# esheldon/ngmix

Measured on AMD Instinct MI355X. Metric: pixel-Gaussian evals/sec (render+loglike), 48×48×6-gauss stamps, 1/2/4/8 GPU, higher is better.
Workload: dtype f64

## Files before the change

### include/ngmix_hip.h

```cpp
#ifndef NGMIX_HIP_H
#define NGMIX_HIP_H

#include <stddef.h>
#include <stdint.h>

#ifdef __cplusplus
extern "C" {
#endif

#define NGMIX_OK 0
#define NGMIX_ERR_DET_TOO_LOW 1
#define NGMIX_ERR_T_TOO_LOW 2
#define NGMIX_ERR_G_RANGE 3
#define NGMIX_ERR_GTOT_ZERO 4
#define NGMIX_ERR_ELOGL_ZERO 5
#define NGMIX_ERR_ZERO_DIV 6
#define NGMIX_ERR_PIXELS_NOT_FILLED 7
#define NGMIX_ERR_HIP (-100)
#define NGMIX_ERR_BAD_ARG (-101)

#define NGMIX_FLAG_CEN_SHIFT 2
#define NGMIX_FLAG_NONPOS_FLUX 4
#define NGMIX_FLAG_NONPOS_SIZE 8
#define NGMIX_FLAG_LOW_DET 16
// ... 110 lines not shown
                            int nmom, double maxrad);
int ngmix_admom(const ngmix_admom_conf *conf, ngmix_gauss2d *wt,
                const ngmix_pixel *pixels, int64_t npix,
                ngmix_admom_result *res);
int ngmix_em_run(int kind, const ngmix_em_conf *conf, ngmix_pixel *pixels,
                 int64_t npix, double *sums, ngmix_gauss2d *gmix, int64_t ngauss,
                 ngmix_gauss2d *gmix_psf, int64_t npsf, ngmix_gauss2d *gmix_conv,
                 int fill_zero_weight, int32_t *numiter, double *frac_diff,
                 double *sky);
int ngmix_deriv_images(const double *gpars, const double *dcov, int64_t ngauss,
                       const double *vv, const double *uu, const double *area,
                       int64_t npix, double *out);


#define NGMIX_STAMP_IGNORE_ZERO_WEIGHT 1

typedef struct {
    int64_t pix_off;
    int32_t nrow, ncol;
    int32_t gm_off;
    int32_t ngauss;
    int32_t flags;
    int32_t npix_kept;
} ngmix_stamp;

#define NGMIX_BATCH_NO_SKIP 1
#define NGMIX_BATCH_EXACT 2
#define NGMIX_BATCH_TRACKED_LOADS 4
#define NGMIX_BATCH_RENDER_OVERWRITE 8

typedef struct {
    int64_t nstamps;
    const ngmix_stamp *stamps;
    const double *val;
    const double *ierr;
    const ngmix_jacobian *jac;
    int32_t max_ngauss;
    int32_t max_npix;
    int32_t any_masked;
    int32_t flags;
    int32_t max_nrow;
    int32_t max_ncol;
} ngmix_batch;

// ... 229 lines not shown
```

### ngmix_amd/_lib.py

```python
import ctypes
import os
import subprocess

import numpy as np

from . import gexceptions

_HERE = os.path.dirname(os.path.abspath(__file__))
_CSRC = os.path.join(_HERE, "csrc")
LIB_PATH = os.environ.get("NGMIX_HIP_LIB", os.path.join(_HERE, "libngmix_hip.so"))

OK = 0
ERR_DET_TOO_LOW = 1
ERR_T_TOO_LOW = 2
ERR_G_RANGE = 3
ERR_GTOT_ZERO = 4
ERR_ELOGL_ZERO = 5
ERR_ZERO_DIV = 6
ERR_PIXELS_NOT_FILLED = 7
ERR_HIP = -100
ERR_BAD_ARG = -101

_RANGE_MESSAGES = {
    ERR_DET_TOO_LOW: "det too low",
    ERR_T_TOO_LOW: "T too low",
    ERR_G_RANGE: "g >= 1",
    ERR_GTOT_ZERO: "gtot == 0",
    ERR_ELOGL_ZERO: "elogL == 0",
}

STAMP_IGNORE_ZERO_WEIGHT = 1
BATCH_NO_SKIP = 1
BATCH_EXACT = 2
BATCH_TRACKED_LOADS = 4
BATCH_RENDER_OVERWRITE = 8

GAUSS2D_DTYPE = np.dtype([
    ("p", "f8"), ("row", "f8"), ("col", "f8"),
    ("irr", "f8"), ("irc", "f8"), ("icc", "f8"), ("det", "f8"),
    ("norm_set", "i8"),
    ("drr", "f8"), ("drc", "f8"), ("dcc", "f8"), ("norm", "f8"), ("pnorm", "f8"),
])
PIXEL_DTYPE = np.dtype([
    ("u", "f8"), ("v", "f8"), ("area", "f8"),
    ("val", "f8"), ("ierr", "f8"), ("fdiff", "f8"),
])
COORD_DTYPE = np.dtype([("u", "f8"), ("v", "f8"), ("area", "f8")])
JACOBIAN_DTYPE = np.dtype([
    ("row0", "f8"), ("col0", "f8"), ("dvdrow", "f8"), ("dvdcol", "f8"),
    ("dudrow", "f8"), ("dudcol", "f8"), ("det", "f8"), ("scale", "f8"),
# ... 338 lines not shown
```

### ngmix_amd/batch.py

```python
import ctypes

import numpy as np

from . import _lib


def _torch():
    import torch
    return torch


def _stream():
    torch = _torch()
    raw = getattr(torch._C, "_cuda_getCurrentRawStream", None)
    if raw is not None:
        return ctypes.c_void_p(raw(torch.cuda.current_device()))
    return ctypes.c_void_p(torch.cuda.current_stream().cuda_stream)


class _on_device(object):

    def __init__(self, dev):
        torch = _torch()
        idx = dev.index if hasattr(dev, "index") else int(dev)
# ... 119 lines not shown
        flat = self.data.detach().cpu().numpy()
        return flat.reshape(-1).view(_lib.GAUSS2D_DTYPE).reshape(
            self.n, self.ngauss).copy()

    def clone(self):
        return GMixBatch(self.data.clone(), self.n, self.ngauss)

    def select(self, index):
        torch = _torch()
        idx = torch.as_tensor(np.ascontiguousarray(index, dtype=np.int64),
                              device=self.device)
        rows = self.data.reshape(self.n, self.ngauss * 13)[idx]
        return GMixBatch(rows.reshape(-1, 13).contiguous(), idx.numel(), self.ngauss)


class StampBatch(object):

    def __init__(self, val, ierr, jac, nrow, ncol, pix_off, ignore_zero_weight,
                 npix_kept=None):
        torch = _torch()
        self.val = val
        self.ierr = ierr
        self.jac = jac
        self.device = ierr.device if ierr is not None else jac.device
        self.n = int(jac.shape[0])
        self.nrow = np.ascontiguousarray(nrow, dtype=np.int32)
        self.ncol = np.ascontiguousarray(ncol, dtype=np.int32)
        self.pix_off = np.ascontiguousarray(pix_off, dtype=np.int64)
        izw = np.broadcast_to(np.asarray(ignore_zero_weight, dtype=bool), (self.n,))
        self.flags = np.where(izw, _lib.STAMP_IGNORE_ZERO_WEIGHT, 0).astype(np.int32)
        self.npix = self.nrow.astype(np.int64) * self.ncol
        self.tracked_loads = False
        self.max_npix = int(self.npix.max()) if self.n else 0
        self.total_pix = int(self.npix.sum())
        self._stamp_tables = {}
        self.npix_kept = self.npix.astype(np.int32).copy()
        if npix_kept is not None:
            self.npix_kept = np.ascontiguousarray(npix_kept, dtype=np.int32)
        elif ierr is not None and self.n:
            tab = self._make_table(self.npix_kept, 0, 0)
            with _on_device(self.device):
                st = _lib.lib().ngmix_count_kept_batch(
                    _dptr(tab), self.n, _dptr(self.ierr), _stream())
            _lib.check(st, "ngmix_count_kept_batch")
            host = tab.cpu().numpy().reshape(-1).view(_lib.STAMP_DTYPE)
            self.npix_kept = host["npix_kept"].copy()
        self.any_masked = bool(np.any(self.npix_kept != self.npix))

    @classmethod
    def from_images(cls, images, weights=None, jacobians=None,
                    ignore_zero_weight=True, device=None):
        torch = _torch()
        dev = _require_cuda(device)
        val = _as_device_f64(images, dev)
        if val.ndim == 2:
            val = val[None]
        n, nrow, ncol = val.shape
        if weights is None:
            ierr = torch.ones_like(val)
        else:
            w = _as_device_f64(weights, dev)
            if w.ndim == 2:
# ... 28 lines not shown
                               [o._ignore_zero_weight for o in obs_list], device=device)

    @classmethod
    def from_arrays(cls, imgs, weights, jac_records, ignore_zero_weight, device=None):
        torch = _torch()
        dev = _require_cuda(device)
        nrow = np.array([im.shape[0] for im in imgs], dtype=np.int32)
        ncol = np.array([im.shape[1] for im in imgs], dtype=np.int32)
        npix = nrow.astype(np.int64) * ncol
        off = np.concatenate([[0], np.cumsum(npix)[:-1]]).astype(np.int64)
        izw = np.array(ignore_zero_weight, dtype=bool)
        tot = int(npix.sum())
        n = len(imgs)
        host = np.empty(2 * tot + 8 * n + 4 * n)
        kept = np.empty(n, dtype=np.int32)
        for i in range(n):
            a, b = int(off[i]), int(off[i] + npix[i])
            host[a:b] = np.asarray(imgs[i], dtype="f8").ravel()
            w = np.asarray(weights[i], dtype="f8").ravel()
            host[tot + a:tot + b] = w
            kept[i] = np.count_nonzero(w > 0.0) if izw[i] else npix[i]
            host[2 * tot + 8 * i:2 * tot + 8 * i + 8] = \
                np.ascontiguousarray(jac_records[i]).view(np.float64).reshape(8)
        tab = np.zeros(n, dtype=_lib.STAMP_DTYPE)
        tab["pix_off"], tab["nrow"], tab["ncol"] = off, nrow, ncol
        tab["gm_off"] = np.arange(n, dtype=np.int32)
        tab["ngauss"] = 1
        tab["flags"] = np.where(izw, _lib.STAMP_IGNORE_ZERO_WEIGHT, 0)
        tab["npix_kept"] = kept
        host[2 * tot + 8 * n:] = tab.view(np.float64)
        dev_all = torch.from_numpy(host).to(dev)
        dval = dev_all[:tot]
        dw = dev_all[tot:2 * tot]
        djac = dev_all[2 * tot:2 * tot + 8 * n].reshape(n, 8)
        dtab = dev_all[2 * tot + 8 * n:].view(torch.int32).reshape(n, 8)
        with _on_device(dev):
            st = _lib.lib().ngmix_weight_to_ierr_batch(
                _dptr(dw), _dptr(dw), dw.numel(), _stream())
        _lib.check(st, "ngmix_weight_to_ierr_batch")
        sb = cls(dval, dw, djac, nrow, ncol, off, izw, npix_kept=kept)
        sb._stamp_tables[1] = dtab
        return sb

    @classmethod
    def from_stacked(cls, images, weights, jac_records, ignore_zero_weight=True,
                     device=None):
        torch = _torch()
        dev = _require_cuda(device)
        if isinstance(images, torch.Tensor):
            ok = (torch.float64, torch.float32)
            assert images.dtype in ok and weights.dtype in ok, "float64 or float32 stamps"
            n, nrow, ncol = images.shape
            assert weights.shape == images.shape, "image and weight must match"
            dval = images.to(dev, non_blocking=True).reshape(-1)
            dw = weights.to(dev, non_blocking=True).reshape(-1)
# ... 14 lines not shown
            return cls(dval, dw, djac, np.full(n, nrow), np.full(n, ncol),
                       np.arange(n, dtype=np.int64) * npix, ignore_zero_weight)
        images = np.asarray(images, dtype="f8")
        weights = np.asarray(weights, dtype="f8")
        n, nrow, ncol = images.shape
        assert weights.shape == images.shape, "image and weight must match"
        npix = nrow * ncol
        tot = n * npix
        jr = np.ascontiguousarray(jac_records)
        if jr.dtype.names is not None:
            jr = jr.view(np.float64)
        jr = jr.reshape(n, 8)
        izw = np.broadcast_to(np.asarray(ignore_zero_weight, dtype=bool), (n,))
        kept = np.where(izw, np.count_nonzero(weights.reshape(n, -1) > 0.0, axis=1),
                        npix).astype(np.int32)
        off = np.arange(n, dtype=np.int64) * npix
        tab = np.zeros(n, dtype=_lib.STAMP_DTYPE)
        tab["pix_off"], tab["nrow"], tab["ncol"] = off, nrow, ncol
        tab["gm_off"] = np.arange(n, dtype=np.int32)
        tab["ngauss"] = 1
        tab["flags"] = np.where(izw, _lib.STAMP_IGNORE_ZERO_WEIGHT, 0)
        tab["npix_kept"] = kept
        host = np.empty(2 * tot + 8 * n + 4 * n)
        host[:tot] = images.reshape(-1)
        host[tot:2 * tot] = weights.reshape(-1)
        host[2 * tot:2 * tot + 8 * n] = jr.reshape(-1)
        host[2 * tot + 8 * n:] = tab.view(np.float64)
        dev_all = torch.from_numpy(host).to(dev)
        dval = dev_all[:tot]
        dw = dev_all[tot:2 * tot]
        djac = dev_all[2 * tot:2 * tot + 8 * n].reshape(n, 8)
        dtab = dev_all[2 * tot + 8 * n:].view(torch.int32).reshape(n, 8)
        with _on_device(dev):
            st = _lib.lib().ngmix_weight_to_ierr_batch(
                _dptr(dw), _dptr(dw), dw.numel(), _stream())
        _lib.check(st, "ngmix_weight_to_ierr_batch")
        sb = cls(dval, dw, djac, np.full(n, nrow), np.full(n, ncol), off, izw, npix_kept=kept)
        sb._stamp_tables[1] = dtab
        return sb

    @classmethod
    def from_observations_geometry(cls, obs_list, device=None):
        dev = _require_cuda(device)
        nrow = np.array([o.image.shape[0] for o in obs_list], dtype=np.int32)
        ncol = np.array([o.image.shape[1] for o in obs_list], dtype=np.int32)
        npix = nrow.astype(np.int64) * ncol
        off = np.concatenate([[0], np.cumsum(npix)[:-1]]).astype(np.int64)
        jac = np.stack([o.jacobian.get_data().view(np.float64).reshape(8)
                        for o in obs_list])
        return cls(None, None, _as_device_f64(jac, dev), nrow, ncol, off, False)

    @staticmethod
# ... 57 lines not shown
        b = _lib.Batch()
        b.nstamps = self.n
        b.stamps = self.stamp_table(ngauss).data_ptr()
        if np.ndim(ngauss) != 0:
            ngauss = int(np.max(ngauss)) if self.n else 0
        b.val = self.val.data_ptr() if self.val is not None else None
        b.ierr = self.ierr.data_ptr() if self.ierr is not None else None
        b.jac = self.jac.data_ptr()
        b.max_ngauss = ngauss
        b.max_npix = self.max_npix
        b.any_masked = int(self.any_masked)
        b.max_nrow = int(self.nrow.max()) if self.n else 0
        b.max_ncol = int(self.ncol.max()) if self.n else 0
        b.flags = (_lib.BATCH_NO_SKIP if no_skip else 0) | \
            (_lib.BATCH_EXACT if exact else 0) | \
            (_lib.BATCH_TRACKED_LOADS if self.tracked_loads else 0)
        return b

    def _packed(self):
        if not hasattr(self, "_packed_layout"):
            start = np.concatenate([[0], np.cumsum(self.npix)[:-1]]) if self.n else \
                np.zeros(0, dtype=np.int64)
            self._packed_layout = bool(np.array_equal(self.pix_off, start))
        return self._packed_layout

    def kept_offsets(self):
        kept = self.npix_kept.astype(np.int64)
        return np.concatenate([[0], np.cumsum(kept)[:-1]]).astype(np.int64)

    def loglike(self, gm, out=None, status=None, no_skip=False, exact=False):
        torch = _torch()
# ... 429 lines not shown
```

### ngmix_amd/csrc/pixpass.hip

```cpp
#include <stdlib.h>

#include <type_traits>

#include "device_utils.hpp"
#include "launch.hpp"

namespace ngmix {

__constant__ double c_exp_table[16] = NGMIX_EXP_TABLE;
__constant__ double c_fexp_coef[12] = NGMIX_FEXP_COEF;

enum PassOp { OP_LOGLIKE = 0, OP_FDIFF = 1, OP_RENDER_FAST = 2,
              OP_RENDER_EXACT = 3, OP_S2N = 4 };

struct GaussLds {
    EvalGauss e;
    PixBox box;
};
static_assert(sizeof(GaussLds) == 64, "GaussLds");

struct LdsLayout {
    double *tab;
    double *red;
    int *ctl;
// ... 290 lines not shown
        "s_mov_b64 %0, exec\n\t"
        "s_and_b64 exec, exec, %3\n\t"
        "global_store_dwordx2 %1, %2, %4\n\t"
        "s_mov_b64 exec, %0"
        : "=&s"(save)
        : "v"(off), "v"(v), "s"(lanes), "s"(base)
        : "scc");
}

__device__ __forceinline__ void gload2_f64_if(double &d0, const void *base0, double &d1,
                                              const void *base1, unsigned off,
                                              int on_mask)
{
    unsigned long long save;
    asm volatile(
        "s_mov_b64 %2, exec\n\t"
        "s_and_b32 exec_lo, exec_lo, %4\n\t"
        "s_and_b32 exec_hi, exec_hi, %4\n\t"
        "global_load_dwordx2 %0, %3, %5\n\t"
        "global_load_dwordx2 %1, %3, %6\n\t"
        "s_mov_b64 exec, %2"
        : "+v"(d0), "+v"(d1), "=&s"(save)
        : "v"(off), "s"(on_mask), "s"(base0), "s"(base1)
        : "scc");
}

template <int N>
__device__ __forceinline__ void wait_vm(double &a, double &b)
{
    asm volatile("s_waitcnt vmcnt(%2)" : "+v"(a), "+v"(b) : "n"(N));
}

__device__ __forceinline__ void wait_vm_all(double &a, double &b, double &c, double &d,
                                            double &e, double &f, double &g, double &h)
{
    asm volatile("s_waitcnt vmcnt(0)"
                 : "+v"(a), "+v"(b), "+v"(c), "+v"(d), "+v"(e), "+v"(f), "+v"(g), "+v"(h));
}

template <int OP, bool MASKED, bool FAST, bool FULL, int TW, bool SKIP>
__device__ __forceinline__ void wave_tiles(
    const LdsLayout &L, const GaussFused *gf, const TileBox *gbox, const TileEnt *te,
    int ng,
    const ngmix_stamp &st, const double *__restrict__ sval,
    const double *__restrict__ sierr, bool masked, double *out, int64_t out_base,
    const ngmix_jacobian &jac, double (&pv)[FUSED_PF], double (&pe)[FUSED_PF],
    double &acc_ll, double &acc_sn, double &acc_sd, const int keep, const TileBox &ub)
{
    constexpr bool kNeedsVal = (OP == OP_LOGLIKE || OP == OP_FDIFF);
    constexpr bool kNeedsIerr = (OP != OP_RENDER_FAST);
    constexpr int TH = WAVE / TW;
    const bool overwrite = keep == 0;
    static_assert(!SKIP || OP == OP_RENDER_FAST, "the line skip is the render's");
    const int lane = threadIdx.x;
    const int lrow = lane / TW, lcol = lane % TW;
    const int nrow = st.nrow, ncol = st.ncol;
    const int ntx = (ncol + TW - 1) / TW;
    const int nty = (nrow + TH - 1) / TH;
    int ntiles = __builtin_amdgcn_readfirstlane(ntx * nty);
    constexpr bool full = FULL;
    const double cen_row = FAST ? gf[0].row : 0.0, cen_col = FAST ? gf[0].col : 0.0;
    const double olv =
// ... 30 lines not shown
    }
    const unsigned long long valid_mask = __builtin_amdgcn_ballot_w64(lane_valid);
    unsigned long long allmask = 0ull;
    int kc = 0;
    const FexpCoef K = load_fexp_coef(c_fexp_coef);

    auto prefetch = [&](int Tn, bool &inb_n, unsigned long long &rm_n, double &nval,
                        double &nierr) {
        if (full) {
            inb_n = true;
            int on;
            asm("s_sub_i32 %0, %1, %2\n\ts_ashr_i32 %0, %0, 31"
                : "=s"(on) : "s"(Tn), "s"(ntiles) : "scc");
            const unsigned off2 = lane_off + (unsigned)te[Tn].off;
            if (kNeedsVal && kNeedsIerr) {
                gload2_f64_if(nval, bval, nierr, bierr, off2, on);
            } else {
                if (kNeedsVal) gload_f64_if(nval, bval, off2, on);
                if (kNeedsIerr) gload_f64_if(nierr, bierr, off2, on);
                if (OP == OP_RENDER_FAST && !SKIP)
                    gload_f64_if(nval, bimg, off2, on & keep);
                if (SKIP) {
                    unsigned long long mr, mc;
                    asm("v_cmp_le_u32 %0, %1, %2"
                        : "=s"(mr)
                        : "v"((unsigned)(te[Tn].r0 + lrow - ub.r_lo)), "s"(ub.r_span));
                    asm("v_cmp_le_u32 %0, %1, %2"
                        : "=s"(mc) : "v"((unsigned)(te[Tn].c0 - ub.c_lo)), "s"(ub.c_span));
                    rm_n = mr & mc;
                    gload_f64_lanes(nval, bimg, off2, rm_n & (unsigned long long)(long long)on);
                }
            }
        } else {
            const int r0n = te[Tn].r0, c0n = te[Tn].c0;
            inb_n = (r0n < rlim) & (c0n < clim);
            if (SKIP)
                inb_n &= ((unsigned)(r0n + lrow - ub.r_lo) <= ub.r_span) &
                         ((unsigned)(c0n - ub.c_lo) <= ub.c_span);
            nval = 0.0;
            nierr = 0.0;
            if (inb_n) {
                const unsigned off2 = lane_off + (unsigned)te[Tn].off;
                if (kNeedsVal) nval = *(const double *)(bval + off2);
                if (kNeedsIerr) nierr = *(const double *)(bierr + off2);
                if (OP == OP_RENDER_FAST && !overwrite) nval = *(const double *)(bimg + off2);
            }
        }
    };

    constexpr int kLoadsPerTile = (kNeedsVal ? 1 : 0) + (kNeedsIerr ? 1 : 0) +
                                  (OP == OP_RENDER_FAST ? 1 : 0);
    auto compute = [&](auto nyounger, int Tc, bool inb, unsigned long long rm, double &pval,
                       double &pierr) {
        const double v = te[Tc].bv + olv, u = te[Tc].bu + olu;
        double dv = v, du = u;
        double v2 = dv * dv, u2 = du * du, vu = dv * du;
        double model = 0.0;

        for (int g0 = 0; g0 < ng; g0 += 32) {
// ... 95 lines not shown
    }
    while (T < ntiles) {
        compute(Y3{}, T, in0, rm0, va0, ie0);
        if (T + 1 < ntiles) compute(Y2{}, T + 1, in1, rm1, va1, ie1);
        prefetch(T + 4, in0, rm0, va0, ie0);
        prefetch(T + 5, in1, rm1, va1, ie1);
        if (T + 2 < ntiles) compute(Y3{}, T + 2, in2, rm2, va2, ie2);
        if (T + 3 < ntiles) compute(Y2{}, T + 3, in3, rm3, va3, ie3);
        prefetch(T + 6, in2, rm2, va2, ie2);
        prefetch(T + 7, in3, rm3, va3, ie3);
        T += 4;
    }
    if (full) wait_vm_all(va0, ie0, va1, ie1, va2, ie2, va3, ie3);
}

template <int OP, bool MASKED, int TW, bool LS = (OP == OP_RENDER_FAST)>
__device__ __forceinline__ void pixpass_wave_body(
    const ngmix_stamp *__restrict__ stamps, const double *__restrict__ val,
    const double *__restrict__ ierr, const ngmix_jacobian *__restrict__ jacs,
    ngmix_gauss2d *gmix, double *out, const int64_t *__restrict__ out_start,
    int32_t *status, int max_ngauss, int nchunks_cap, int no_skip, int tile_cap)
{
    extern __shared__ __attribute__((aligned(16))) char smem[];
    const LdsLayout L = carve(smem, max_ngauss, nchunks_cap, tile_cap);
    GaussFused *gf = (GaussFused *)L.gl;
    TileBox *gbox = (TileBox *)(gf + max_ngauss);
    TileEnt *te = (TileEnt *)L.tb;

    const int s = blockIdx.x;
    const ngmix_stamp st = stamps[s];
    const ngmix_jacobian jac = jacs[s];
    const int nrow = st.nrow, ncol = st.ncol, ng = st.ngauss;
    const int npix = nrow * ncol;
    ngmix_gauss2d *gm = gmix + st.gm_off;
    const double *sval = val + st.pix_off;
    const double *sierr = ierr + st.pix_off;
    const bool izw = (st.flags & NGMIX_STAMP_IGNORE_ZERO_WEIGHT) != 0;
    constexpr bool kNeedsVal = (OP == OP_LOGLIKE || OP == OP_FDIFF);
    const double area = jac.scale * jac.scale;
    const int lane = threadIdx.x;

    constexpr int TH = WAVE / TW;
    const int ntx = (ncol + TW - 1) / TW;
    const int nty = (nrow + TH - 1) / TH;
    const int ntiles = ntx * nty;
    for (int T = lane; T < ntiles + FUSED_SENTINELS; T += WAVE) {
        TileEnt e;
        if (T < ntiles) {
            const int ty = T / ntx, tx = T - ty * ntx;
            e.r0 = ty * TH;
            e.c0 = tx * TW;
            const double rd = (double)e.r0 - jac.row0, cd = (double)e.c0 - jac.col0;
            e.bv = fma(jac.dvdrow, rd, jac.dvdcol * cd);
            e.bu = fma(jac.dudrow, rd, jac.dudcol * cd);
            e.off = (e.r0 * ncol + e.c0) * 8;
// ... 19 lines not shown
    const int keep = (OP == OP_RENDER_FAST && !LS) ? (((no_skip >> 2) & 1) - 1) : -1;
    const bool full = (nrow % TH) == 0 && (ncol % TW) == 0 && !(no_skip & 2);
    double pv[FUSED_PF], pe[FUSED_PF];
#pragma unroll
    for (int t = 0; t < FUSED_PF; t++) {
        pv[t] = 0.0;
        pe[t] = 0.0;
    }
    if (full && ng > 0 && ntiles > 0 && !LS) {
        const unsigned lane_off = (unsigned)((lane / TW) * ncol + lane % TW) * 8u;
#pragma unroll
        for (int t = 0; t < FUSED_PF; t++) {
            const int on = __builtin_amdgcn_readfirstlane(-(int)(t < ntiles));
            const unsigned off = lane_off + (unsigned)te[t].off;
            if (kNeedsVal) gload_f64_if(pv[t], (const char *)sval, off, on);
            if (OP != OP_RENDER_FAST) gload_f64_if(pe[t], (const char *)sierr, off, on);
            if (OP == OP_RENDER_FAST)
                gload_f64_if(pv[t], (const char *)(out + st.pix_off), off, on & keep);
        }
    }

    const bool overwrite = OP == OP_RENDER_FAST && !LS && (no_skip & 4);
    const int stcode = lazy_norms<WAVE>(L, gm, ng);
    if (stcode != NGMIX_OK || (overwrite && ng == 0)) {
        asm volatile("s_waitcnt vmcnt(0)" ::: "memory");
        if (overwrite)
            for (int p = lane; p < npix; p += WAVE) out[st.pix_off + p] = 0.0;
        if (lane == 0) status[s] = stcode;
        return;
    }
    if (lane < 16) L.tab[lane] = c_exp_table[15 - lane];
// ... 32 lines not shown
        un.cmin = ubx[2];
        un.cmax = ubx[3];
        const TileBox t = tile_box(un, 1, TW);
        ub.r_lo = __builtin_amdgcn_readfirstlane(t.r_lo);
        ub.r_span = (unsigned)__builtin_amdgcn_readfirstlane((int)t.r_span);
        ub.c_lo = __builtin_amdgcn_readfirstlane(t.c_lo);
        ub.c_span = (unsigned)__builtin_amdgcn_readfirstlane((int)t.c_span);
    }
    const bool masked = MASKED && izw && st.npix_kept != npix;
    if (OP == OP_FDIFF && masked) build_rank_tables<WAVE>(L.cmask, L.cpre, sierr, npix);
    const int64_t out_base = (OP == OP_FDIFF) ? out_start[s] : 0;

    double acc_ll = 0.0, acc_sn = 0.0, acc_sd = 0.0;
    if (ng > 0) {
        if (fast && full)
            wave_tiles<OP, MASKED, true, true, TW, LS>(L, gf, gbox, te, ng, st, sval, sierr, masked,
                out, out_base, jac, pv, pe, acc_ll, acc_sn, acc_sd, keep, ub);
        else if (fast)
            wave_tiles<OP, MASKED, true, false, TW, LS>(L, gf, gbox, te, ng, st, sval, sierr, masked,
                out, out_base, jac, pv, pe, acc_ll, acc_sn, acc_sd, keep, ub);
        else if (full)
            wave_tiles<OP, MASKED, false, true, TW, LS>(L, gf, gbox, te, ng, st, sval, sierr, masked,
                out, out_base, jac, pv, pe, acc_ll, acc_sn, acc_sd, keep, ub);
        else
            wave_tiles<OP, MASKED, false, false, TW, LS>(L, gf, gbox, te, ng, st, sval, sierr, masked,
                out, out_base, jac, pv, pe, acc_ll, acc_sn, acc_sd, keep, ub);
    } else if (OP != OP_RENDER_FAST) {
        for (int p = lane; p < npix; p += WAVE) {
            const double pv = kNeedsVal ? sval[p] : 0.0, pe = sierr[p];
            if (masked && !(pe > 0.0)) continue;
            if (OP == OP_LOGLIKE) acc_ll = fma(pv * pv, pe * pe, acc_ll);
            if (OP == OP_FDIFF) {
                const int rank = masked ? kept_rank(L.cmask, L.cpre, p) : p;
                out[out_base + rank] = (0.0 - pv) * pe;
            }
        }
    }

    if (OP == OP_LOGLIKE) {
        double *red = L.red;
        const double r0_ = row16_total(acc_ll), r1_ = row16_total(acc_sn),
// ... 45 lines not shown
{
    pixpass_wave_body<OP, MASKED, TW, false>(stamps, val, ierr, jacs, gmix, out, out_start,
                                             status, max_ngauss, nchunks_cap, no_skip, tile_cap);
}

template <int OP, bool MASKED, int TW>
__global__ __launch_bounds__(WAVE) __attribute__((amdgpu_waves_per_eu(7, 7)))
void pixpass_wave_kernel7(
    const ngmix_stamp *__restrict__ stamps, const double *__restrict__ val,
    const double *__restrict__ ierr, const ngmix_jacobian *__restrict__ jacs,
    ngmix_gauss2d *gmix, double *out, const int64_t *__restrict__ out_start,
    int32_t *status, int max_ngauss, int nchunks_cap, int no_skip, int tile_cap)
{
    pixpass_wave_body<OP, MASKED, TW>(stamps, val, ierr, jacs, gmix, out, out_start, status,
                                      max_ngauss, nchunks_cap, no_skip, tile_cap);
}


constexpr int FUSED_TILE_CAP = 2048;

static int pick_k(int max_npix)
{
    if (max_npix <= 32 * 32) return 4;
    return 9;
}

template <int OP>
static int launch_grid(const ngmix_batch *b, ngmix_gauss2d *gmix, double *out,
                       const int64_t *out_start, int32_t *status, void *stream)
{
// ... 39 lines not shown
               : OP == OP_S2N   ? "pixpass_grid_kernel<s2n>"
                                : "pixpass_grid_kernel<render>");
        NGMIX_HIP_CHECK(hipLaunchKernel(kern, grid, block, args, lds, s));
        return NGMIX_OK;
    }
    constexpr int FOP = (OP == OP_RENDER_EXACT) ? OP_RENDER_FAST : OP;
    const bool mk = b->any_masked && FOP != OP_RENDER_FAST;
    const void *kern = mk ? (const void *)pixpass_wave_kernel<FOP, true, TW>
                          : (const void *)pixpass_wave_kernel<FOP, false, TW>;
    if (FOP == OP_RENDER_FAST && (no_skip & 4))
        kern = (const void *)pixpass_wave_kernel_plain<OP_RENDER_FAST, false, 16>;
    static const bool six_waves = getenv("NGMIX_LOGLIKE_6WAVES") != nullptr;
    if (FOP == OP_LOGLIKE && !six_waves)
        kern = mk ? (const void *)pixpass_wave_kernel7<OP_LOGLIKE, true, 8>
                  : (const void *)pixpass_wave_kernel7<OP_LOGLIKE, false, 8>;
    const size_t flds = lds_bytes(max_ng, nchunks_cap, a_tc);
    if (flds > 160 * 1024) {
        set_last_error_msg("stamp needs more than 160 KiB of LDS");
        return NGMIX_ERR_BAD_ARG;
    }
    if (flds > 64 * 1024)
        NGMIX_HIP_CHECK(hipFuncSetAttribute(
            kern, hipFuncAttributeMaxDynamicSharedMemorySize, (int)flds));
    dim3 grid((unsigned)b->nstamps), block(WAVE);
    void *args[] = {&a_stamps, &a_val, &a_ierr, &a_jac, &gmix, &out, &out_start,
                    &status, &a_ng, &a_nc, &a_ns, &a_tc};
    census(FOP == OP_LOGLIKE ? (six_waves ? "pixpass_wave_kernel<loglike>"
                                          : "pixpass_wave_kernel7<loglike>")
           : FOP == OP_FDIFF ? "pixpass_wave_kernel<fdiff>"
           : FOP == OP_S2N   ? "pixpass_wave_kernel<s2n>"
// ... 259 lines not shown
    for (int64_t i = blockIdx.x * (int64_t)BLOCK + threadIdx.x; i < n;
         i += (int64_t)gridDim.x * BLOCK) {
        double ivar = w ? w[i] : 1.0;
        if (ivar < 0.0) ivar = 0.0;
        ierr[i] = sqrt(ivar);
    }
}

__global__ __launch_bounds__(BLOCK) void count_kept_kernel(ngmix_stamp *stamps,
                                                          const double *ierr)
{
    __shared__ double red[16];
    ngmix_stamp st = stamps[blockIdx.x];
    const int npix = st.nrow * st.ncol;
    const bool izw = (st.flags & NGMIX_STAMP_IGNORE_ZERO_WEIGHT) != 0;
    double cnt = 0.0;
    for (int p = threadIdx.x; p < npix; p += BLOCK)
        if (!izw || ierr[st.pix_off + p] > 0.0) cnt += 1.0;
    double v[1] = {cnt};
    block_sum<1>(v, red);
    if (threadIdx.x == 0) stamps[blockIdx.x].npix_kept = (int)v[0];
}

__global__ __launch_bounds__(BLOCK) void fastexp_kernel(const double *__restrict__ x,
                                                         double *__restrict__ out, int64_t n,
                                                         int which)
{
    __shared__ double tab[16];
    if (threadIdx.x < 16) tab[threadIdx.x] = c_exp_table[threadIdx.x];
    __syncthreads();
    for (int64_t i = blockIdx.x * (int64_t)BLOCK + threadIdx.x; i < n;
         i += (int64_t)gridDim.x * BLOCK) {
        const double v = x[i];
        out[i] = which == 0 ? fexp(v, tab) : (which == 1 ? apod_window(v) : apod_window_deriv(v));
    }
}
// ... 81 lines not shown
```

### ngmix_amd/csrc/store.hip

```cpp
#include <dlfcn.h>
#include <rccl/rccl.h>
#include <stdint.h>
#include <string.h>

#include <new>
#include <vector>

#include "common.hpp"
#include "launch.hpp"

namespace ngmix {

struct Store {
    ngmix_batch b;
    std::vector<ngmix_stamp> host_stamps;
    int64_t total_pix;
    double *d_val, *d_ierr;
    ngmix_jacobian *d_jac;
    ngmix_stamp *d_stamps;
    int device;
};

struct Rccl {
    void *handle = nullptr;
// ... 137 lines not shown
int ngmix_batch_upload(ngmix_batch *b, const double *images, const double *weights,
                       const ngmix_jacobian *jac, void *stream)
{
    if (!b || !images || !jac) {
        set_last_error_msg("ngmix_batch_upload: bad argument");
        return NGMIX_ERR_BAD_ARG;
    }
    Store *s = (Store *)b;
    hipStream_t q = (hipStream_t)stream;
    const size_t pixbytes = (size_t)s->total_pix * sizeof(double);
    const size_t n = (size_t)b->nstamps;
    if (n == 0) return NGMIX_OK;
    NGMIX_HIP_CHECK(hipMemcpyAsync(s->d_val, images, pixbytes, hipMemcpyHostToDevice, q));
    NGMIX_HIP_CHECK(hipMemcpyAsync(s->d_jac, jac, n * sizeof(ngmix_jacobian),
                                   hipMemcpyHostToDevice, q));
    for (size_t i = 0; i < n; i++)
        s->host_stamps[i].npix_kept = s->host_stamps[i].nrow * s->host_stamps[i].ncol;
    NGMIX_HIP_CHECK(hipMemcpyAsync(s->d_stamps, s->host_stamps.data(),
                                   n * sizeof(ngmix_stamp), hipMemcpyHostToDevice, q));
    if (weights) {
        NGMIX_HIP_CHECK(hipMemcpyAsync(s->d_ierr, weights, pixbytes,
                                       hipMemcpyHostToDevice, q));
        int st = launch_weight_to_ierr(s->d_ierr, s->d_ierr, s->total_pix, q);
        if (st) return st;
        st = launch_count_kept(s->d_stamps, b->nstamps, s->d_ierr, q);
        if (st) return st;
        NGMIX_HIP_CHECK(hipMemcpyAsync(s->host_stamps.data(), s->d_stamps,
                                       n * sizeof(ngmix_stamp), hipMemcpyDeviceToHost, q));
    } else {
        int st = launch_weight_to_ierr(nullptr, s->d_ierr, s->total_pix, q);
        if (st) return st;
    }
    NGMIX_HIP_CHECK(hipStreamSynchronize(q));
    int32_t masked = 0;
    for (size_t i = 0; i < n; i++) {
        const ngmix_stamp &st = s->host_stamps[i];
        if (st.npix_kept != st.nrow * st.ncol) masked = 1;
        if ((st.flags & NGMIX_STAMP_IGNORE_ZERO_WEIGHT) && st.npix_kept == 0) {
            set_last_error_msg("ngmix_batch_upload: a stamp has no positive weight");
            return NGMIX_ERR_BAD_ARG;
        }
    }
    b->any_masked = masked;
    return NGMIX_OK;
}

int ngmix_batch_npix_kept(const ngmix_batch *b, int32_t *npix_kept)
{
    if (!b || !npix_kept) return NGMIX_ERR_BAD_ARG;
    const Store *s = (const Store *)b;
    for (size_t i = 0; i < s->host_stamps.size(); i++)
        npix_kept[i] = s->host_stamps[i].npix_kept;
    return NGMIX_OK;
}

int ngmix_batch_free(ngmix_batch *b)
{
    if (!b) return NGMIX_OK;
// ... 64 lines not shown
```

Baseline: 2057 billion.

## Detect uniform-weight stamps and load only one ierr value per stamp

Stamps whose inverse-error values are all bitwise identical are now flagged as uniform, either on the host or in the count-kept kernel. For those stamps the pixel-pass kernels mask the ierr address offset to zero, so every lane reads the same element instead of streaming a full ierr plane from memory. Batches with no uniform stamps dispatch to separate kernel instantiations that keep the original streaming path. The cost is an extra scan over the weights at upload time, additional kernel variants, and a dependence on the weights staying uniform after upload.

```diff
diff --git a/include/ngmix_hip.h b/include/ngmix_hip.h
--- a/include/ngmix_hip.h
+++ b/include/ngmix_hip.h
@@ -148,6 +148,7 @@
 
 
 #define NGMIX_STAMP_IGNORE_ZERO_WEIGHT 1
+#define NGMIX_STAMP_UNIFORM_IERR 2
 
 typedef struct {
     int64_t pix_off;
@@ -162,6 +163,7 @@
 #define NGMIX_BATCH_EXACT 2
 #define NGMIX_BATCH_TRACKED_LOADS 4
 #define NGMIX_BATCH_RENDER_OVERWRITE 8
+#define NGMIX_BATCH_STREAM_IERR 16
 
 typedef struct {
     int64_t nstamps;
diff --git a/ngmix_amd/_lib.py b/ngmix_amd/_lib.py
--- a/ngmix_amd/_lib.py
+++ b/ngmix_amd/_lib.py
@@ -30,10 +30,12 @@
 }
 
 STAMP_IGNORE_ZERO_WEIGHT = 1
+STAMP_UNIFORM_IERR = 2
 BATCH_NO_SKIP = 1
 BATCH_EXACT = 2
 BATCH_TRACKED_LOADS = 4
 BATCH_RENDER_OVERWRITE = 8
+BATCH_STREAM_IERR = 16
 
 GAUSS2D_DTYPE = np.dtype([
     ("p", "f8"), ("row", "f8"), ("col", "f8"),
diff --git a/ngmix_amd/batch.py b/ngmix_amd/batch.py
--- a/ngmix_amd/batch.py
+++ b/ngmix_amd/batch.py
@@ -157,10 +157,26 @@
         return GMixBatch(rows.reshape(-1, 13).contiguous(), idx.numel(), self.ngauss)
 
 
+def _uniform_weights(w):
+    w = np.ascontiguousarray(w, dtype=np.float64)
+    n = w.shape[0]
+    if w.shape[1] == 0:
+        return np.zeros(n, dtype=bool)
+    bits = w.view(np.int64)
+    first = w[:, 0]
+    with np.errstate(invalid="ignore"):
+        ok = (first > 0.0) & np.isfinite(first)
+    step = max(1, (1 << 22) // w.shape[1])
+    for a in range(0, n, step):
+        blk = bits[a:a + step]
+        ok[a:a + step] &= np.all(blk == blk[:, :1], axis=1)
+    return ok
+
+
 class StampBatch(object):
 
     def __init__(self, val, ierr, jac, nrow, ncol, pix_off, ignore_zero_weight,
-                 npix_kept=None):
+                 npix_kept=None, uniform_ierr=None):
         torch = _torch()
         self.val = val
         self.ierr = ierr
@@ -174,13 +190,25 @@
         self.flags = np.where(izw, _lib.STAMP_IGNORE_ZERO_WEIGHT, 0).astype(np.int32)
         self.npix = self.nrow.astype(np.int64) * self.ncol
         self.tracked_loads = False
+        self.stream_ierr = False
         self.max_npix = int(self.npix.max()) if self.n else 0
         self.total_pix = int(self.npix.sum())
         self._stamp_tables = {}
         self.npix_kept = self.npix.astype(np.int32).copy()
         if npix_kept is not None:
             self.npix_kept = np.ascontiguousarray(npix_kept, dtype=np.int32)
-        elif ierr is not None and self.n:
+            if uniform_ierr is not None:
+                self.flags |= np.where(np.asarray(uniform_ierr, dtype=bool),
+                                       _lib.STAMP_UNIFORM_IERR, 0).astype(np.int32)
+            self.any_masked = bool(np.any(self.npix_kept != self.npix))
+            self.any_uniform = bool(np.any(self.flags & _lib.STAMP_UNIFORM_IERR))
+        else:
+            self.rescan_weights()
+
+    def rescan_weights(self):
+        self.flags = self.flags & ~np.int32(_lib.STAMP_UNIFORM_IERR)
+        self.npix_kept = self.npix.astype(np.int32).copy()
+        if self.ierr is not None and self.n:
             tab = self._make_table(self.npix_kept, 0, 0)
             with _on_device(self.device):
                 st = _lib.lib().ngmix_count_kept_batch(
@@ -188,7 +216,10 @@
             _lib.check(st, "ngmix_count_kept_batch")
             host = tab.cpu().numpy().reshape(-1).view(_lib.STAMP_DTYPE)
             self.npix_kept = host["npix_kept"].copy()
+            self.flags = host["flags"].copy()
         self.any_masked = bool(np.any(self.npix_kept != self.npix))
+        self.any_uniform = bool(np.any(self.flags & _lib.STAMP_UNIFORM_IERR))
+        self._stamp_tables = {}
 
     @classmethod
     def from_images(cls, images, weights=None, jacobians=None,
@@ -247,19 +278,22 @@
         n = len(imgs)
         host = np.empty(2 * tot + 8 * n + 4 * n)
         kept = np.empty(n, dtype=np.int32)
+        uniform = np.empty(n, dtype=bool)
         for i in range(n):
             a, b = int(off[i]), int(off[i] + npix[i])
             host[a:b] = np.asarray(imgs[i], dtype="f8").ravel()
             w = np.asarray(weights[i], dtype="f8").ravel()
             host[tot + a:tot + b] = w
             kept[i] = np.count_nonzero(w > 0.0) if izw[i] else npix[i]
+            uniform[i] = _uniform_weights(w[None])[0]
             host[2 * tot + 8 * i:2 * tot + 8 * i + 8] = \
                 np.ascontiguousarray(jac_records[i]).view(np.float64).reshape(8)
         tab = np.zeros(n, dtype=_lib.STAMP_DTYPE)
         tab["pix_off"], tab["nrow"], tab["ncol"] = off, nrow, ncol
         tab["gm_off"] = np.arange(n, dtype=np.int32)
         tab["ngauss"] = 1
-        tab["flags"] = np.where(izw, _lib.STAMP_IGNORE_ZERO_WEIGHT, 0)
+        tab["flags"] = np.where(izw, _lib.STAMP_IGNORE_ZERO_WEIGHT, 0) | \
+            np.where(uniform, _lib.STAMP_UNIFORM_IERR, 0)
         tab["npix_kept"] = kept
         host[2 * tot + 8 * n:] = tab.view(np.float64)
         dev_all = torch.from_numpy(host).to(dev)
@@ -271,7 +305,8 @@
             st = _lib.lib().ngmix_weight_to_ierr_batch(
                 _dptr(dw), _dptr(dw), dw.numel(), _stream())
         _lib.check(st, "ngmix_weight_to_ierr_batch")
-        sb = cls(dval, dw, djac, nrow, ncol, off, izw, npix_kept=kept)
+        sb = cls(dval, dw, djac, nrow, ncol, off, izw, npix_kept=kept,
+                 uniform_ierr=uniform)
         sb._stamp_tables[1] = dtab
         return sb
 
@@ -316,12 +351,14 @@
         izw = np.broadcast_to(np.asarray(ignore_zero_weight, dtype=bool), (n,))
         kept = np.where(izw, np.count_nonzero(weights.reshape(n, -1) > 0.0, axis=1),
                         npix).astype(np.int32)
+        uniform = _uniform_weights(weights.reshape(n, -1))
         off = np.arange(n, dtype=np.int64) * npix
         tab = np.zeros(n, dtype=_lib.STAMP_DTYPE)
         tab["pix_off"], tab["nrow"], tab["ncol"] = off, nrow, ncol
         tab["gm_off"] = np.arange(n, dtype=np.int32)
         tab["ngauss"] = 1
-        tab["flags"] = np.where(izw, _lib.STAMP_IGNORE_ZERO_WEIGHT, 0)
+        tab["flags"] = np.where(izw, _lib.STAMP_IGNORE_ZERO_WEIGHT, 0) | \
+            np.where(uniform, _lib.STAMP_UNIFORM_IERR, 0)
         tab["npix_kept"] = kept
         host = np.empty(2 * tot + 8 * n + 4 * n)
         host[:tot] = images.reshape(-1)
@@ -337,7 +374,8 @@
             st = _lib.lib().ngmix_weight_to_ierr_batch(
                 _dptr(dw), _dptr(dw), dw.numel(), _stream())
         _lib.check(st, "ngmix_weight_to_ierr_batch")
-        sb = cls(dval, dw, djac, np.full(n, nrow), np.full(n, ncol), off, izw, npix_kept=kept)
+        sb = cls(dval, dw, djac, np.full(n, nrow), np.full(n, ncol), off, izw, npix_kept=kept,
+                 uniform_ierr=uniform)
         sb._stamp_tables[1] = dtab
         return sb
 
@@ -425,7 +463,8 @@
         b.max_ncol = int(self.ncol.max()) if self.n else 0
         b.flags = (_lib.BATCH_NO_SKIP if no_skip else 0) | \
             (_lib.BATCH_EXACT if exact else 0) | \
-            (_lib.BATCH_TRACKED_LOADS if self.tracked_loads else 0)
+            (_lib.BATCH_TRACKED_LOADS if self.tracked_loads else 0) | \
+            (_lib.BATCH_STREAM_IERR if self.stream_ierr or not self.any_uniform else 0)
         return b
 
     def _packed(self):
diff --git a/ngmix_amd/csrc/pixpass.hip b/ngmix_amd/csrc/pixpass.hip
--- a/ngmix_amd/csrc/pixpass.hip
+++ b/ngmix_amd/csrc/pixpass.hip
@@ -328,14 +328,34 @@
 {
     unsigned long long save;
     asm volatile(
-        "s_mov_b64 %2, exec\n\t"
-        "s_and_b32 exec_lo, exec_lo, %4\n\t"
-        "s_and_b32 exec_hi, exec_hi, %4\n\t"
-        "global_load_dwordx2 %0, %3, %5\n\t"
-        "global_load_dwordx2 %1, %3, %6\n\t"
-        "s_mov_b64 exec, %2"
-        : "+v"(d0), "+v"(d1), "=&s"(save)
-        : "v"(off), "s"(on_mask), "s"(base0), "s"(base1)
+        "s_mov_b64 %[save], exec\n\t"
+        "s_and_b32 exec_lo, exec_lo, %[on]\n\t"
+        "s_and_b32 exec_hi, exec_hi, %[on]\n\t"
+        "global_load_dwordx2 %[d0], %[off], %[b0]\n\t"
+        "global_load_dwordx2 %[d1], %[off], %[b1]\n\t"
+        "s_mov_b64 exec, %[save]"
+        : [d0] "+v"(d0), [d1] "+v"(d1), [save] "=&s"(save)
+        : [off] "v"(off), [on] "s"(on_mask), [b0] "s"(base0), [b1] "s"(base1)
+        : "scc");
+}
+
+__device__ __forceinline__ void gload2_f64_if(double &d0, const void *base0, double &d1,
+                                              const void *base1, unsigned off,
+                                              int on_mask, int on1_mask)
+{
+    unsigned long long save;
+    asm volatile(
+        "s_mov_b64 %[save], exec\n\t"
+        "s_and_b32 exec_lo, exec_lo, %[on]\n\t"
+        "s_and_b32 exec_hi, exec_hi, %[on]\n\t"
+        "global_load_dwordx2 %[d0], %[off], %[b0]\n\t"
+        "s_and_b32 exec_lo, exec_lo, %[on1]\n\t"
+        "s_and_b32 exec_hi, exec_hi, %[on1]\n\t"
+        "global_load_dwordx2 %[d1], %[off], %[b1]\n\t"
+        "s_mov_b64 exec, %[save]"
+        : [d0] "+v"(d0), [d1] "+v"(d1), [save] "=&s"(save)
+        : [off] "v"(off), [on] "s"(on_mask), [b0] "s"(base0), [b1] "s"(base1),
+          [on1] "s"(on1_mask)
         : "scc");
 }
 
@@ -352,14 +372,15 @@
                  : "+v"(a), "+v"(b), "+v"(c), "+v"(d), "+v"(e), "+v"(f), "+v"(g), "+v"(h));
 }
 
-template <int OP, bool MASKED, bool FAST, bool FULL, int TW, bool SKIP>
+template <int OP, bool MASKED, bool FAST, bool FULL, int TW, bool SKIP, bool UE>
 __device__ __forceinline__ void wave_tiles(
     const LdsLayout &L, const GaussFused *gf, const TileBox *gbox, const TileEnt *te,
     int ng,
     const ngmix_stamp &st, const double *__restrict__ sval,
     const double *__restrict__ sierr, bool masked, double *out, int64_t out_base,
     const ngmix_jacobian &jac, double (&pv)[FUSED_PF], double (&pe)[FUSED_PF],
-    double &acc_ll, double &acc_sn, double &acc_sd, const int keep, const TileBox &ub)
+    double &acc_ll, double &acc_sn, double &acc_sd, const int keep, const TileBox &ub,
+    const int ie_on)
 {
     constexpr bool kNeedsVal = (OP == OP_LOGLIKE || OP == OP_FDIFF);
     constexpr bool kNeedsIerr = (OP != OP_RENDER_FAST);
@@ -420,10 +441,11 @@
                 : "=s"(on) : "s"(Tn), "s"(ntiles) : "scc");
             const unsigned off2 = lane_off + (unsigned)te[Tn].off;
             if (kNeedsVal && kNeedsIerr) {
-                gload2_f64_if(nval, bval, nierr, bierr, off2, on);
+                if (UE) gload2_f64_if(nval, bval, nierr, bierr, off2, on, ie_on);
+                else gload2_f64_if(nval, bval, nierr, bierr, off2, on);
             } else {
                 if (kNeedsVal) gload_f64_if(nval, bval, off2, on);
-                if (kNeedsIerr) gload_f64_if(nierr, bierr, off2, on);
+                if (kNeedsIerr) gload_f64_if(nierr, bierr, off2, on & ie_on);
                 if (OP == OP_RENDER_FAST && !SKIP)
                     gload_f64_if(nval, bimg, off2, on & keep);
                 if (SKIP) {
@@ -448,7 +470,7 @@
             if (inb_n) {
                 const unsigned off2 = lane_off + (unsigned)te[Tn].off;
                 if (kNeedsVal) nval = *(const double *)(bval + off2);
-                if (kNeedsIerr) nierr = *(const double *)(bierr + off2);
+                if (kNeedsIerr) nierr = *(const double *)(bierr + (off2 & (unsigned)ie_on));
                 if (OP == OP_RENDER_FAST && !overwrite) nval = *(const double *)(bimg + off2);
             }
         }
@@ -574,7 +596,7 @@
     if (full) wait_vm_all(va0, ie0, va1, ie1, va2, ie2, va3, ie3);
 }
 
-template <int OP, bool MASKED, int TW, bool LS = (OP == OP_RENDER_FAST)>
+template <int OP, bool MASKED, int TW, bool LS = (OP == OP_RENDER_FAST), bool UE = true>
 __device__ __forceinline__ void pixpass_wave_body(
     const ngmix_stamp *__restrict__ stamps, const double *__restrict__ val,
     const double *__restrict__ ierr, const ngmix_jacobian *__restrict__ jacs,
@@ -599,6 +621,9 @@
     constexpr bool kNeedsVal = (OP == OP_LOGLIKE || OP == OP_FDIFF);
     const double area = jac.scale * jac.scale;
     const int lane = threadIdx.x;
+    static_assert(NGMIX_STAMP_UNIFORM_IERR == 2, "the shift below");
+    constexpr bool ue = UE && OP != OP_RENDER_FAST;
+    const int ie_on = ue ? ((__builtin_amdgcn_readfirstlane(st.flags) >> 1) & 1) - 1 : -1;
 
     constexpr int TH = WAVE / TW;
     const int ntx = (ncol + TW - 1) / TW;
@@ -648,7 +673,8 @@
             const int on = __builtin_amdgcn_readfirstlane(-(int)(t < ntiles));
             const unsigned off = lane_off + (unsigned)te[t].off;
             if (kNeedsVal) gload_f64_if(pv[t], (const char *)sval, off, on);
-            if (OP != OP_RENDER_FAST) gload_f64_if(pe[t], (const char *)sierr, off, on);
+            if (OP != OP_RENDER_FAST)
+                gload_f64_if(pe[t], (const char *)sierr, off & (unsigned)ie_on, on);
             if (OP == OP_RENDER_FAST)
                 gload_f64_if(pv[t], (const char *)(out + st.pix_off), off, on & keep);
         }
@@ -711,17 +737,17 @@
     double acc_ll = 0.0, acc_sn = 0.0, acc_sd = 0.0;
     if (ng > 0) {
         if (fast && full)
-            wave_tiles<OP, MASKED, true, true, TW, LS>(L, gf, gbox, te, ng, st, sval, sierr, masked,
-                out, out_base, jac, pv, pe, acc_ll, acc_sn, acc_sd, keep, ub);
+            wave_tiles<OP, MASKED, true, true, TW, LS, ue>(L, gf, gbox, te, ng, st, sval, sierr, masked,
+                out, out_base, jac, pv, pe, acc_ll, acc_sn, acc_sd, keep, ub, ie_on);
         else if (fast)
-            wave_tiles<OP, MASKED, true, false, TW, LS>(L, gf, gbox, te, ng, st, sval, sierr, masked,
-                out, out_base, jac, pv, pe, acc_ll, acc_sn, acc_sd, keep, ub);
+            wave_tiles<OP, MASKED, true, false, TW, LS, ue>(L, gf, gbox, te, ng, st, sval, sierr, masked,
+                out, out_base, jac, pv, pe, acc_ll, acc_sn, acc_sd, keep, ub, ie_on);
         else if (full)
-            wave_tiles<OP, MASKED, false, true, TW, LS>(L, gf, gbox, te, ng, st, sval, sierr, masked,
-                out, out_base, jac, pv, pe, acc_ll, acc_sn, acc_sd, keep, ub);
+            wave_tiles<OP, MASKED, false, true, TW, LS, ue>(L, gf, gbox, te, ng, st, sval, sierr, masked,
+                out, out_base, jac, pv, pe, acc_ll, acc_sn, acc_sd, keep, ub, ie_on);
         else
-            wave_tiles<OP, MASKED, false, false, TW, LS>(L, gf, gbox, te, ng, st, sval, sierr, masked,
-                out, out_base, jac, pv, pe, acc_ll, acc_sn, acc_sd, keep, ub);
+            wave_tiles<OP, MASKED, false, false, TW, LS, ue>(L, gf, gbox, te, ng, st, sval, sierr, masked,
+                out, out_base, jac, pv, pe, acc_ll, acc_sn, acc_sd, keep, ub, ie_on);
     } else if (OP != OP_RENDER_FAST) {
         for (int p = lane; p < npix; p += WAVE) {
             const double pv = kNeedsVal ? sval[p] : 0.0, pe = sierr[p];
@@ -797,6 +823,31 @@
 {
     pixpass_wave_body<OP, MASKED, TW>(stamps, val, ierr, jacs, gmix, out, out_start, status,
                                       max_ngauss, nchunks_cap, no_skip, tile_cap);
+}
+
+template <int OP, bool MASKED, int TW>
+__global__ __launch_bounds__(WAVE) void pixpass_wave_kernel_stream(
+    const ngmix_stamp *__restrict__ stamps, const double *__restrict__ val,
+    const double *__restrict__ ierr, const ngmix_jacobian *__restrict__ jacs,
+    ngmix_gauss2d *gmix, double *out, const int64_t *__restrict__ out_start,
+    int32_t *status, int max_ngauss, int nchunks_cap, int no_skip, int tile_cap)
+{
+    pixpass_wave_body<OP, MASKED, TW, false, false>(stamps, val, ierr, jacs, gmix, out,
+                                                    out_start, status, max_ngauss,
+                                                    nchunks_cap, no_skip, tile_cap);
+}
+
+template <int OP, bool MASKED, int TW>
+__global__ __launch_bounds__(WAVE) __attribute__((amdgpu_waves_per_eu(7, 7)))
+void pixpass_wave_kernel7_stream(
+    const ngmix_stamp *__restrict__ stamps, const double *__restrict__ val,
+    const double *__restrict__ ierr, const ngmix_jacobian *__restrict__ jacs,
+    ngmix_gauss2d *gmix, double *out, const int64_t *__restrict__ out_start,
+    int32_t *status, int max_ngauss, int nchunks_cap, int no_skip, int tile_cap)
+{
+    pixpass_wave_body<OP, MASKED, TW, false, false>(stamps, val, ierr, jacs, gmix, out,
+                                                    out_start, status, max_ngauss,
+                                                    nchunks_cap, no_skip, tile_cap);
 }
 
 
@@ -866,6 +917,15 @@
     if (FOP == OP_LOGLIKE && !six_waves)
         kern = mk ? (const void *)pixpass_wave_kernel7<OP_LOGLIKE, true, 8>
                   : (const void *)pixpass_wave_kernel7<OP_LOGLIKE, false, 8>;
+    if constexpr (FOP != OP_RENDER_FAST) {
+        if (b->flags & NGMIX_BATCH_STREAM_IERR) {
+            kern = mk ? (const void *)pixpass_wave_kernel_stream<FOP, true, TW>
+                      : (const void *)pixpass_wave_kernel_stream<FOP, false, TW>;
+            if (FOP == OP_LOGLIKE && !six_waves)
+                kern = mk ? (const void *)pixpass_wave_kernel7_stream<OP_LOGLIKE, true, 8>
+                          : (const void *)pixpass_wave_kernel7_stream<OP_LOGLIKE, false, 8>;
+        }
+    }
     const size_t flds = lds_bytes(max_ng, nchunks_cap, a_tc);
     if (flds > 160 * 1024) {
         set_last_error_msg("stamp needs more than 160 KiB of LDS");
@@ -1155,12 +1215,22 @@
     ngmix_stamp st = stamps[blockIdx.x];
     const int npix = st.nrow * st.ncol;
     const bool izw = (st.flags & NGMIX_STAMP_IGNORE_ZERO_WEIGHT) != 0;
-    double cnt = 0.0;
-    for (int p = threadIdx.x; p < npix; p += BLOCK)
-        if (!izw || ierr[st.pix_off + p] > 0.0) cnt += 1.0;
-    double v[1] = {cnt};
-    block_sum<1>(v, red);
-    if (threadIdx.x == 0) stamps[blockIdx.x].npix_kept = (int)v[0];
+    const long long first = npix > 0 ? __double_as_longlong(ierr[st.pix_off]) : 0ll;
+    double cnt = 0.0, ndiff = 0.0;
+    for (int p = threadIdx.x; p < npix; p += BLOCK) {
+        const double e = ierr[st.pix_off + p];
+        if (!izw || e > 0.0) cnt += 1.0;
+        if (__double_as_longlong(e) != first) ndiff += 1.0;
+    }
+    double v[2] = {cnt, ndiff};
+    block_sum<2>(v, red);
+    if (threadIdx.x == 0) {
+        const double f = __longlong_as_double(first);
+        const bool uniform = npix > 0 && v[1] == 0.0 && f > 0.0 && f < HUGE_VAL;
+        stamps[blockIdx.x].npix_kept = (int)v[0];
+        stamps[blockIdx.x].flags = (st.flags & ~NGMIX_STAMP_UNIFORM_IERR) |
+                                   (uniform ? NGMIX_STAMP_UNIFORM_IERR : 0);
+    }
 }
 
 __global__ __launch_bounds__(BLOCK) void fastexp_kernel(const double *__restrict__ x,
diff --git a/ngmix_amd/csrc/store.hip b/ngmix_amd/csrc/store.hip
--- a/ngmix_amd/csrc/store.hip
+++ b/ngmix_amd/csrc/store.hip
@@ -175,8 +175,10 @@
     NGMIX_HIP_CHECK(hipMemcpyAsync(s->d_val, images, pixbytes, hipMemcpyHostToDevice, q));
     NGMIX_HIP_CHECK(hipMemcpyAsync(s->d_jac, jac, n * sizeof(ngmix_jacobian),
                                    hipMemcpyHostToDevice, q));
-    for (size_t i = 0; i < n; i++)
+    for (size_t i = 0; i < n; i++) {
         s->host_stamps[i].npix_kept = s->host_stamps[i].nrow * s->host_stamps[i].ncol;
+        s->host_stamps[i].flags &= ~NGMIX_STAMP_UNIFORM_IERR;
+    }
     NGMIX_HIP_CHECK(hipMemcpyAsync(s->d_stamps, s->host_stamps.data(),
                                    n * sizeof(ngmix_stamp), hipMemcpyHostToDevice, q));
     if (weights) {
@@ -191,18 +193,24 @@
     } else {
         int st = launch_weight_to_ierr(nullptr, s->d_ierr, s->total_pix, q);
         if (st) return st;
+        st = launch_count_kept(s->d_stamps, b->nstamps, s->d_ierr, q);
+        if (st) return st;
+        NGMIX_HIP_CHECK(hipMemcpyAsync(s->host_stamps.data(), s->d_stamps,
+                                       n * sizeof(ngmix_stamp), hipMemcpyDeviceToHost, q));
     }
     NGMIX_HIP_CHECK(hipStreamSynchronize(q));
-    int32_t masked = 0;
+    int32_t masked = 0, uniform = 0;
     for (size_t i = 0; i < n; i++) {
         const ngmix_stamp &st = s->host_stamps[i];
         if (st.npix_kept != st.nrow * st.ncol) masked = 1;
+        if (st.flags & NGMIX_STAMP_UNIFORM_IERR) uniform = 1;
         if ((st.flags & NGMIX_STAMP_IGNORE_ZERO_WEIGHT) && st.npix_kept == 0) {
             set_last_error_msg("ngmix_batch_upload: a stamp has no positive weight");
             return NGMIX_ERR_BAD_ARG;
         }
     }
     b->any_masked = masked;
+    b->flags = (b->flags & ~NGMIX_BATCH_STREAM_IERR) | (uniform ? 0 : NGMIX_BATCH_STREAM_IERR);
     return NGMIX_OK;
 }
 
```

Measured after the change: 2276 billion (median of 6 runs). +10.7%, better.
